# Duankaiwen/LSNet

Measured on AMD Instinct MI355X. Metric: img/s train LSNet R-50-FPN 1333x800 bs2/GPU, higher is better.
Workload: dtype f32 (fp32-equivalent: 6 bf16 MFMA terms per product on exact 3-way operand splits, fp32 accumulate); 1 GPU; LSNet R50-FPN bbox (conv_module_type=dcn), 2 img/GPU 3x800x1344 (1333x800 padded to /32), 7 gt/img, fwd+bwd+gradient arena (the reducer's buckets, no collective on one rank)+clip35+SGD; global_batch=2, parallelism=dp1, world_size=1, memory_format=channels_last, launch=eager

## Files before the change

include/lsnet_hip.h:

```cpp
#ifndef LSNET_HIP_H_
#define LSNET_HIP_H_

#include <stdint.h>

#ifdef __cplusplus
extern "C" {
#endif

typedef struct ihipStream_t *lsn_stream_t;

typedef enum {
    LSN_OK = 0,
    LSN_ERR_INVALID = -1,
    LSN_ERR_UNSUPPORTED = -2,
    LSN_ERR_RUNTIME = -3
} lsn_status;

typedef enum { LSN_NCHW = 0, LSN_NHWC = 1 } lsn_layout;

typedef struct { int64_t b, c, h, w; } lsn_strides4;

typedef struct {
    int B, C, H, W;
    int Co, Ho, Wo;
// ... 245 lines not shown

int lsn_bn_eval_act_forward(const float *x, const float *residual, float *y, const float *running_mean,
                            const float *running_var, const float *gamma, const float *beta, float eps, int relu,
                            int N, int C, lsn_stream_t stream);
int64_t lsn_bn_eval_act_workspace_bytes(int N, int C);
int lsn_bn_eval_act_backward(const float *grad_y, const float *y, const float *x, const float *running_mean,
                             const float *running_var, const float *gamma, float eps, int relu, float *grad_x,
                             float *grad_residual, float *grad_gamma, float *grad_beta, void *workspace, int N,
                             int C, int accumulate, lsn_stream_t stream);
int lsn_relu_gate(const float *grad_y, const float *y, float *grad, int64_t n, lsn_stream_t stream);
typedef struct lsn_gate_job {
    const float *grad_y, *y;
    float *grad;
    int B;
    int64_t per_image, gy_batch_stride;
} lsn_gate_job;
int lsn_relu_gate_multi(int n_jobs, const lsn_gate_job *jobs, lsn_stream_t stream);

enum {
    LSN_DBG_BLOCK_MASK = 0xffff,
    LSN_DBG_ANCHOR_ONE_WAVE = 1 << 20,
    LSN_DBG_FWD_SK_ALWAYS = 1 << 21,
    LSN_DBG_FWD_SK_NEVER = 1 << 22,
    LSN_DBG_ATOMIC_SCATTER = 1 << 23,
    LSN_DBG_WG_COMPUTED_TAPS = 1 << 24,
    LSN_DBG_WG_SCALAR_LOADS = 1 << 25,
    LSN_DBG_GENERAL_GEMMS = 1 << 28
};
int lsn_debug_phase_clocks(long long *device_buf_512, int word);

typedef struct lsn_prof_entry {
    char name[48];
    long long launches;
    double total_ms;
    double flops;
    double bytes;
} lsn_prof_entry;
int lsn_prof_enable(int on);
int lsn_prof_read(lsn_prof_entry *out, int max_entries);

typedef struct lsn_prof_launch {
    int kind, C, Co, kh, kw, stride, pad, dil, relu, xpitch, n_levels, has_residual, has_gate;
    int B[16], H[16], W[16];
    float ms;
} lsn_prof_launch;
int lsn_prof_launch_log(int on);
int lsn_prof_read_launches(lsn_prof_launch *out, int max_entries);

int lsn_scratch_stats(long long *out4);

int lsn_wgrad_defer(int max_mbytes, lsn_stream_t stream);
int lsn_wgrad_flush(lsn_stream_t stream);

int lsn_selftest_mfma(const float *A, const float *B, float *D, int M, int N, int K, int variant,
                      lsn_stream_t stream);

int lsn_image_prep_u8(const uint8_t *src, int sh, int sw, int c, int dh, int dw, int flip_h, int flip_v,
                      const float *mean, const float *inv_std, int reverse_channels, float pad_val, float *dst,
                      int out_h, int out_w, lsn_stream_t stream);

int lsn_cross_iou_bbox_forward(const float *pred, const float *target, const uint8_t *active, const float *anchor,
                               const float *bbox_gt, const float *weight, int64_t n, float alpha, float eps,
                               float *loss_rows, lsn_stream_t stream);
int lsn_cross_iou_bbox_backward(const float *pred, const float *target, const uint8_t *active, const float *anchor,
                                const float *bbox_gt, const float *weight, const float *grad_rows, int64_t n,
                                float alpha, float eps, float *grad_pred, lsn_stream_t stream);

int lsn_cross_iou_bbox_stage_forward(const float *pred_raw, const float *gt_pts, const float *anchor3, const float *bbox_gt,
                                     const float *weight, int64_t n, float base_scale, float alpha, float eps,
                                     float *loss_rows, lsn_stream_t stream);
int lsn_cross_iou_bbox_stage_backward(const float *pred_raw, const float *gt_pts, const float *anchor3, const float *bbox_gt,
                                      const float *weight, const float *grad_rows, int64_t n, float base_scale, float alpha,
                                      float eps, float *grad_raw, lsn_stream_t stream);

int lsn_cross_iou_rows_forward(int kind, const float *pred, const float *target, const uint8_t *active, const float *anchor,
                               const float *bbox_gt, const float *vs, const float *weight, int64_t n, int ncomp, int sub,
                               float alpha, float eps, float *loss_rows, lsn_stream_t stream);
int lsn_cross_iou_rows_backward(int kind, const float *pred, const float *target, const uint8_t *active, const float *anchor,
                                const float *bbox_gt, const float *vs, const float *weight, const float *grad_rows, int64_t n,
                                int ncomp, int sub, float alpha, float eps, float *grad_pred, lsn_stream_t stream);

int lsn_pool_output_size(int in, int k, int stride, int pad, int ceil_mode);
int lsn_max_pool2d_forward(const float *x, int x_pitch, float *y, int y_pitch, uint8_t *slot, int B, int H, int W, int C, int kh,
                           int kw, int stride, int pad, lsn_stream_t stream);
int lsn_max_pool2d_backward(const float *grad_y, int gy_pitch, const uint8_t *slot, float *grad_x, int gx_pitch, int B, int H, int W,
                            int C, int kh, int kw, int stride, int pad, lsn_stream_t stream);

int lsn_avg_pool2d_forward(const float *x, int x_pitch, float *y, int y_pitch, int B, int H, int W, int C, int kh, int kw, int stride,
                           int pad, int ceil_mode, int count_include_pad, lsn_stream_t stream);
int lsn_avg_pool2d_backward(const float *grad_y, int gy_pitch, float *grad_x, int gx_pitch, int B, int H, int W, int C, int kh, int kw,
                            int stride, int pad, int ceil_mode, int count_include_pad, lsn_stream_t stream);

int lsn_upsample_add_forward(const float *top, int top_pitch, const float *lat, int lat_pitch, float *out, int out_pitch, int B, int h,
                             int w, int H, int W, int C, lsn_stream_t stream);
int lsn_upsample_add_backward(const float *grad_out, int go_pitch, float *grad_top, int gt_pitch, int accumulate, int B, int h, int w,
                              int H, int W, int C, lsn_stream_t stream);

int lsn_corner_pool_forward(int mode, const float *x, int x_pitch, float *y, int y_pitch, int accumulate, int B, int H, int W, int C,
                            lsn_stream_t stream);
int lsn_corner_pool_backward(int mode, const float *x, int x_pitch, const float *grad_y, int gy_pitch, float *grad_x, int gx_pitch,
                             int accumulate, int B, int H, int W, int C, lsn_stream_t stream);

#ifdef __cplusplus
}
#endif
#endif
// ... 1 lines not shown
```

lsnet_amd/_lib.py:

```python
import ctypes
import os

_HERE = os.path.dirname(os.path.abspath(__file__))
SO_PATH = os.environ.get('LSNET_HIP_SO') or os.path.join(_HERE, 'csrc', 'liblsnet_hip.so')

c_float_p = ctypes.POINTER(ctypes.c_float)
c_i64_p = ctypes.POINTER(ctypes.c_int64)


class Strides4(ctypes.Structure):
    _fields_ = [('b', ctypes.c_int64), ('c', ctypes.c_int64), ('h', ctypes.c_int64), ('w', ctypes.c_int64)]


class DcnShape(ctypes.Structure):
    _fields_ = [('B', ctypes.c_int), ('C', ctypes.c_int), ('H', ctypes.c_int), ('W', ctypes.c_int),
                ('Co', ctypes.c_int), ('Ho', ctypes.c_int), ('Wo', ctypes.c_int),
                ('kh', ctypes.c_int), ('kw', ctypes.c_int), ('stride', ctypes.c_int), ('pad', ctypes.c_int),
                ('dil', ctypes.c_int), ('groups', ctypes.c_int), ('deformable_groups', ctypes.c_int),
                ('scale_h', ctypes.c_float), ('scale_w', ctypes.c_float), ('mask_is_logit', ctypes.c_int),
                ('workspace', ctypes.c_void_p), ('gather_workspace', ctypes.c_void_p),
                ('gather_workspace_bytes', ctypes.c_int64), ('accumulate_param_grads', ctypes.c_int),
                ('out_pitch', ctypes.c_int), ('weights_prepared', ctypes.c_int)]


# ... 28 lines not shown


class ConvLevel(ctypes.Structure):
    _fields_ = [('x', ctypes.c_void_p), ('out', ctypes.c_void_p), ('grad_out', ctypes.c_void_p),
                ('B', ctypes.c_int), ('H', ctypes.c_int), ('W', ctypes.c_int), ('residual', ctypes.c_void_p),
                ('gate', ctypes.c_void_p)]


class ConvWprep(ctypes.Structure):
    _fields_ = [('kind', ctypes.c_int), ('w', ctypes.c_void_p), ('prepared', ctypes.c_void_p), ('C', ctypes.c_int),
                ('Co', ctypes.c_int), ('kh', ctypes.c_int), ('kw', ctypes.c_int), ('stride', ctypes.c_int),
                ('pad', ctypes.c_int), ('dil', ctypes.c_int),
                ('bn_gamma', ctypes.c_void_p), ('bn_var', ctypes.c_void_p), ('bn_beta', ctypes.c_void_p),
                ('bn_mean', ctypes.c_void_p), ('shift_out', ctypes.c_void_p), ('bn_eps', ctypes.c_float)]


class GnLevel(ctypes.Structure):
    _fields_ = [('x', ctypes.c_void_p), ('y', ctypes.c_void_p), ('dy', ctypes.c_void_p), ('dx', ctypes.c_void_p),
                ('B', ctypes.c_int), ('HW', ctypes.c_int), ('y_batch_stride', ctypes.c_longlong),
                ('dy_batch_stride', ctypes.c_longlong)]


class GateJob(ctypes.Structure):
    _fields_ = [('grad_y', ctypes.c_void_p), ('y', ctypes.c_void_p), ('grad', ctypes.c_void_p), ('B', ctypes.c_int),
                ('per_image', ctypes.c_int64), ('gy_batch_stride', ctypes.c_int64)]


class ProfEntry(ctypes.Structure):
    _fields_ = [('name', ctypes.c_char * 48), ('launches', ctypes.c_longlong), ('total_ms', ctypes.c_double),
                ('flops', ctypes.c_double), ('bytes', ctypes.c_double)]


class ProfLaunch(ctypes.Structure):
    _fields_ = [(k, ctypes.c_int) for k in ('kind', 'C', 'Co', 'kh', 'kw', 'stride', 'pad', 'dil', 'relu', 'xpitch', 'n_levels',
                                            'has_residual', 'has_gate')] + \
               [('B', ctypes.c_int * 16), ('H', ctypes.c_int * 16), ('W', ctypes.c_int * 16), ('ms', ctypes.c_float)]


EXPORTS = [
    'lsn_last_error', 'lsn_version', 'lsn_dcn_forward', 'lsn_dcn_backward', 'lsn_dcn_backward_workspace_bytes', 'lsn_dcn_pitched_ok', 'lsn_dcn_prepared_ok',
    'lsn_deform_conv_forward', 'lsn_deform_conv_backward_input', 'lsn_deform_conv_backward_parameters',
    'lsn_modulated_deform_conv_forward', 'lsn_modulated_deform_conv_backward',
    'lsn_pyramid_deform_conv_forward', 'lsn_pyramid_deform_conv_backward_input',
    'lsn_pyramid_deform_conv_backward_parameters',
    'lsn_sigmoid_focal_loss_forward', 'lsn_sigmoid_focal_loss_backward', 'lsn_sigmoid_focal_loss_sum',
    'lsn_sigmoid_focal_loss_backward_weighted', 'lsn_sigmoid_focal_loss_level_sums', 'lsn_sigmoid_focal_loss_backward_levels',
    'lsn_level_sums', 'lsn_level_expand',
    'lsn_nms_workspace_bytes', 'lsn_nms', 'lsn_topk_columns', 'lsn_offset_chain_forward', 'lsn_offset_chain_backward', 'lsn_clip_sgd_workspace_bytes', 'lsn_clip_sgd_step', 'lsn_selftest_mfma', 'lsn_debug_phase_clocks',
    'lsn_prof_enable', 'lsn_prof_read', 'lsn_prof_launch_log', 'lsn_prof_read_launches', 'lsn_scratch_stats', 'lsn_wgrad_defer', 'lsn_wgrad_flush',
    'lsn_group_norm_workspace_bytes', 'lsn_group_norm_forward', 'lsn_group_norm_backward',
    'lsn_set_math_mode', 'lsn_get_math_mode', 'lsn_conv2d_forward', 'lsn_conv2d_forward_pitched', 'lsn_conv2d_backward_data',
    'lsn_conv2d_prepared_bytes', 'lsn_conv2d_prepare_weights', 'lsn_conv2d_prepare_weights_multi',
    'lsn_conv2d_prepare_weights_item',
    'lsn_conv2d_forward_prepared',
    'lsn_conv2d_backward_data_prepared',
    'lsn_conv2d_forward_multi', 'lsn_conv2d_backward_data_multi', 'lsn_conv2d_backward_weight_multi', 'lsn_conv2d_backward_weight',
    'lsn_grouped_conv2d_forward', 'lsn_grouped_conv2d_backward_data', 'lsn_grouped_conv2d_backward_weight',
    'lsn_bn_eval_act_forward', 'lsn_bn_eval_act_backward', 'lsn_bn_eval_act_workspace_bytes',
    'lsn_relu_gate', 'lsn_relu_gate_multi', 'lsn_conv2d_backward_weight_bn', 'lsn_conv2d_backward_weight_bn_jobs',
    'lsn_image_prep_u8', 'lsn_cross_iou_bbox_forward', 'lsn_cross_iou_bbox_backward',
    'lsn_cross_iou_bbox_stage_forward', 'lsn_cross_iou_bbox_stage_backward',
    'lsn_cross_iou_rows_forward', 'lsn_cross_iou_rows_backward',
    'lsn_assign_workspace_bytes', 'lsn_centroid_assign', 'lsn_centroid_assign_batch', 'lsn_atss_assign', 'lsn_atss_assign_batch',
    'lsn_dense_targets',
    'lsn_pool_output_size', 'lsn_max_pool2d_forward', 'lsn_max_pool2d_backward', 'lsn_avg_pool2d_forward', 'lsn_avg_pool2d_backward',
    'lsn_upsample_add_forward', 'lsn_upsample_add_backward', 'lsn_corner_pool_forward', 'lsn_corner_pool_backward',
]

_lib = None


def load():
    global _lib
    if _lib is not None:
        return _lib
    if not os.path.exists(SO_PATH):
        raise RuntimeError(
            f'{SO_PATH} is missing: build it with `python -c "import __graft_entry__ as g; g.build()"` '
            '(hipcc --offload-arch=gfx950). lsnet_amd has no fallback path.')
    lib = ctypes.CDLL(SO_PATH)
    lib.lsn_last_error.restype = ctypes.c_char_p
    lib.lsn_nms_workspace_bytes.restype = ctypes.c_int64
    lib.lsn_assign_workspace_bytes.restype = ctypes.c_int64
    lib.lsn_group_norm_workspace_bytes.restype = ctypes.c_int64
    lib.lsn_bn_eval_act_workspace_bytes.restype = ctypes.c_int64
    lib.lsn_dcn_backward_workspace_bytes.restype = ctypes.c_int64
    lib.lsn_clip_sgd_workspace_bytes.restype = ctypes.c_int64
    lib.lsn_conv2d_prepared_bytes.restype = ctypes.c_int64
    for name in EXPORTS:
        getattr(lib, name)
    _lib = lib
    return lib


def check(rc):
    if rc != 0:
        msg = load().lsn_last_error().decode('utf-8', 'replace')
        if rc == -2:
            raise NotImplementedError(msg)
        raise RuntimeError(msg)


PROF_FAMILIES = ('dcn_fwd', 'dcn_bwd_data', 'dcn_wgrad', 'conv_fwd', 'conv_bwd_data', 'conv_wgrad', 'norm', 'gconv')


def prof_enable(on, families=None):
    mask = 0
    if on:
        mask = 1 if families is None else sum(1 << PROF_FAMILIES.index(f) for f in families)
        if mask == 1 and families is not None:
            mask |= 1 << 31
    check(load().lsn_prof_enable(mask))


def prof_read():
    arr = (ProfEntry * 16)()
    n = load().lsn_prof_read(arr, 16)
    if n < 0:
        check(n)
    return {arr[i].name.decode(): dict(launches=int(arr[i].launches), total_ms=arr[i].total_ms,
                                       flops=arr[i].flops, bytes=arr[i].bytes) for i in range(n)}


def wgrad_defer(max_mbytes, stream=None):
    import ctypes
    import torch
    st = ctypes.c_void_p(torch.cuda.current_stream().cuda_stream if stream is None else stream)
    check(load().lsn_wgrad_defer(int(max_mbytes), st))


def wgrad_flush(stream=None):
    import ctypes
    import torch
    st = ctypes.c_void_p(torch.cuda.current_stream().cuda_stream if stream is None else stream)
    check(load().lsn_wgrad_flush(st))


def scratch_stats():
    import ctypes
    out = (ctypes.c_longlong * 4)()
    check(load().lsn_scratch_stats(out))
    return dict(mallocs=int(out[0]), held_bytes=int(out[1]), blocking_syncs=int(out[2]), pool_allocs=int(out[3]))


DBG_BLOCK_MASK = 0xffff
DBG_ANCHOR_ONE_WAVE = 1 << 20
DBG_FWD_SK_ALWAYS = 1 << 21
DBG_FWD_SK_NEVER = 1 << 22
DBG_ATOMIC_SCATTER = 1 << 23
DBG_WG_COMPUTED_TAPS = 1 << 24
DBG_WG_SCALAR_LOADS = 1 << 25
DBG_GENERAL_GEMMS = 1 << 28


def set_debug_word(word, buf=None):
    check(load().lsn_debug_phase_clocks(None if buf is None else ctypes.c_void_p(buf), ctypes.c_int(word)))


MATH_FP32, MATH_BF16X3, MATH_BF16X6, MATH_BF16 = 0, 1, 2, 3
_MODES = {'fp32': MATH_FP32, 'bf16x3': MATH_BF16X3, 'bf16x6': MATH_BF16X6, 'bf16': MATH_BF16}


def set_math_mode(mode):
    check(load().lsn_set_math_mode(_MODES[mode] if isinstance(mode, str) else mode))


def get_math_mode():
    m = load().lsn_get_math_mode()
    return {v: k for k, v in _MODES.items()}[m]


def split_math():
    return get_math_mode() != 'fp32'
```

lsnet_amd/csrc/build.py:

```python
import os
import shutil
import subprocess
import sys

HERE = os.path.dirname(os.path.abspath(__file__))
SO = os.path.join(HERE, 'liblsnet_hip.so')
SOURCES = ['dcn.hip', 'misc.hip', 'norm.hip', 'conv.hip', 'gconv.hip', 'image.hip', 'loss.hip', 'assign.hip', 'pool.hip']
HEADERS = ['common.h', 'dcn_kernels.h', 'dcn_gather_kernels.h', 'dcn_grouped_kernels.h', 'conv_kernels.h', 'conv_wgrad_kernels.h', 'dcn_mm_kernels.h', 'prof.h', 'cross_iou_row.h', 'assign_rows.h', 'pool_rows.h', os.path.join('..', '..', 'include', 'lsnet_hip.h')]
FLAGS = ['--offload-arch=gfx950', '-O3', '-std=c++17', '-fPIC', '-shared', '-ffp-contract=fast',
         '-fno-slp-vectorize', '-Wno-unused-result']


def kernel_signature():
    import hashlib
    h = hashlib.sha256()
    for f in ('common.h', 'conv_kernels.h', 'conv_wgrad_kernels.h', 'conv.hip', 'dcn_kernels.h', 'dcn_gather_kernels.h', 'dcn_mm_kernels.h', 'dcn_grouped_kernels.h', 'dcn.hip'):
        with open(os.path.join(HERE, f), 'rb') as fh:
            h.update(fh.read())
    return h.hexdigest()[:16]


def _hipcc():
    for c in (shutil.which('hipcc'), '/opt/rocm/bin/hipcc'):
        if c and os.path.exists(c):
            return c
    raise RuntimeError('hipcc not found: liblsnet_hip.so cannot be built')


OBJ_DIR = os.path.join(HERE, 'build')
UNIT_HEADERS = {
    'dcn.hip': ['common.h', 'dcn_kernels.h', 'dcn_gather_kernels.h', 'dcn_mm_kernels.h', 'dcn_grouped_kernels.h', 'conv_kernels.h', 'prof.h'],
    'conv.hip': ['common.h', 'conv_kernels.h', 'conv_wgrad_kernels.h', 'prof.h'],
    'misc.hip': ['common.h', 'prof.h'], 'norm.hip': ['common.h', 'prof.h'], 'gconv.hip': ['common.h', 'prof.h'],
    'image.hip': ['common.h'], 'loss.hip': ['common.h', 'cross_iou_row.h'], 'assign.hip': ['common.h', 'assign_rows.h'],
    'pool.hip': ['common.h', 'pool_rows.h'],
}
UNIT_FLAGS = {'assign.hip': ['-ffp-contract=off']}
API_HEADER = os.path.join('..', '..', 'include', 'lsnet_hip.h')


def _stale(target, deps):
    if not os.path.exists(target):
        return True
    t = os.path.getmtime(target)
    return any(os.path.exists(d) and os.path.getmtime(d) > t for d in deps)


def _unit_deps(src):
    return [os.path.join(HERE, f) for f in [src] + UNIT_HEADERS.get(src, HEADERS) + [API_HEADER]] + [os.path.abspath(__file__)]


def needs_build(so=None, obj_dir=None):
    so = so or SO
    obj_dir = obj_dir or OBJ_DIR
    if not os.path.exists(so):
        return True
    return any(_stale(os.path.join(obj_dir, s + '.o'), _unit_deps(s)) for s in SOURCES) or \
        _stale(so, [os.path.join(obj_dir, s + '.o') for s in SOURCES])


def build(force=False, verbose=False, defines=(), so=None):
    so = so or SO
    obj_dir = OBJ_DIR if so == SO else so + '.build'
    if not force and not needs_build(so, obj_dir):
        return so
    os.makedirs(obj_dir, exist_ok=True)
    cc = _hipcc()
    cflags = [f for f in FLAGS if f != '-shared'] + ['-D' + d for d in defines]
    jobs = []
    for s in SOURCES:
        obj = os.path.join(obj_dir, s + '.o')
        if force or _stale(obj, _unit_deps(s)):
            cmd = [cc] + cflags + UNIT_FLAGS.get(s, []) + ['-c', os.path.join(HERE, s), '-o', obj]
            if verbose:
                print(' '.join(cmd), file=sys.stderr)
            jobs.append((s, subprocess.Popen(cmd, cwd=HERE)))
    failed = [s for s, p in jobs if p.wait() != 0]
    if failed:
        raise RuntimeError('hipcc failed for ' + ', '.join(failed))
    cmd = [cc, '--offload-arch=gfx950', '-shared', '-fPIC'] + [os.path.join(obj_dir, s + '.o') for s in SOURCES] + ['-o', so]
    if verbose:
        print(' '.join(cmd), file=sys.stderr)
    subprocess.check_call(cmd, cwd=HERE)
    return so

# ... 26 lines not shown
```

lsnet_amd/csrc/conv.hip:

```cpp
#include <hip/hip_runtime.h>
#include <stdint.h>
#include <stdlib.h>
#include <string.h>

#include <vector>

#include "../../include/lsnet_hip.h"
#include "common.h"
#include "conv_kernels.h"
#include "conv_wgrad_kernels.h"
#include "prof.h"

namespace lsn {

int split_np();
static int conv_np()
{
    switch (split_np()) {
    case 0: return 6;
    case 1: return 1;
    case 3: return 3;
    case 6: return 6;
    default: return -1;
    }
}
static int conv_npl() { return split_npl(conv_np()); }

static long long g_stat[4] = {0, 0, 0, 0};
void lib_stat(int which, long long add) { g_stat[which & 3] += add; }

struct Scratch {
    hipStream_t st;
    float *p;
    size_t floats;
};
static Scratch g_scr[16];
static int g_nscr = 0;
struct RJob {
    bool fold;
    const float *part, *part_b;
    float *gw, *gb;
    size_t n;
    int nb, splits, splits_b, R, Co;
    WgFold f;
};
struct Arena {
    hipStream_t st;
    float *p;
    size_t floats, used;
    long long defer_mb;
    std::vector<RJob> *jobs;
};
static Arena g_arena[16];
static int g_narena = 0;
static Arena *arena_of(hipStream_t st, bool create)
{
    for (int i = 0; i < g_narena; ++i)
        if (g_arena[i].st == st) return &g_arena[i];
    if (!create || g_narena == 16) return nullptr;
    g_arena[g_narena] = Arena{st, nullptr, 0, 0, 0, new std::vector<RJob>()};
    return &g_arena[g_narena++];
}
// ... 170 lines not shown
            LSN_HIP(hipFuncSetAttribute(reinterpret_cast<const void *>(k), hipFuncAttributeMaxDynamicSharedMemorySize, (int)lds));
            attr_set = true;
        }
        hipLaunchKernelGGL(k, grid, dim3(256), lds, st, a);
    } else {
        auto k = conv_mm_kernel<TM, TN, WM, WN, NP, UNAL, FINE, TRANS, false>;
        static bool attr_set = false;
        if (!attr_set) {
            LSN_HIP(hipFuncSetAttribute(reinterpret_cast<const void *>(k), hipFuncAttributeMaxDynamicSharedMemorySize, (int)lds));
            attr_set = true;
        }
        hipLaunchKernelGGL(k, grid, dim3(256), lds, st, a);
    }
    if (ks > 1) {
        const int blocks = (int)((n / 4 + 255) / 256 < 1024 ? (n / 4 + 255) / 256 : 1024);
        const size_t o = (size_t)pix0 * a.Co;
        hipLaunchKernelGGL(conv_splitk_reduce_kernel, dim3(blocks > 0 ? blocks : 1), dim3(256), 0, st, a.part, a.lv[0].out + o, a.bias,
                           a.lv[0].res ? a.lv[0].res + o : nullptr, a.lv[0].gate ? a.lv[0].gate + o : nullptr, (int)n, a.Co, ks,
                           a.relu);
    }
    LSN_HIP(hipGetLastError());
    return 0;
}

template <int TM, int TN, int WM, int WN, int NP, bool UNAL, bool FINE, bool TRANS = false>
static int launch_conv_cfg(ConvArgs &a, int ks, hipStream_t st)
{
    constexpr int BM = WM * TM * 32, BN = WN * TN * 32;
    int tiles = 0;
    for (int i = 0; i < a.nlv; ++i) {
        a.lv[i].tile0 = tiles;
        tiles += (a.lv[i].P + BM - 1) / BM;
    }
    a.ntiles = tiles;
    return launch_conv_range<TM, TN, WM, WN, NP, UNAL, FINE, TRANS>(a, ks, 0, tiles, st);
}

template <int TM, int TN, int WM, int WN, bool FINE>
static int launch_conv(ConvArgs &a, int ks, hipStream_t st)
{
    if constexpr (TN == 2 && WN == 2) {
        if (a.C % 4 != 0 || a.xpitch % 4 != 0)
            return split_dispatch(conv_np(), [&](auto np) {
                return launch_conv_cfg<TM, TN, WM, WN, decltype(np)::value, true, false>(a, ks, st);
            });
    }
    if (a.C % 4 != 0 || a.xpitch % 4 != 0)
        return fail(LSN_ERR_UNSUPPORTED, "conv2d: C %% 4 != 0 needs more than 64 output channels");
    return split_dispatch(conv_np(), [&](auto np) {
        return launch_conv_cfg<TM, TN, WM, WN, decltype(np)::value, false, FINE>(a, ks, st);
    });
}

static int conv_forward(ConvArgs &a, hipStream_t st)
{
    auto blocks = [&](int bm, int bn) {
        int t = 0;
        for (int i = 0; i < a.nlv; ++i) t += (a.lv[i].P + bm - 1) / bm;
        return t * ((a.Co + bn - 1) / bn);
    };
    int cfg;
    if (a.Co <= 32) cfg = 4;
    else if (a.Co <= 64) cfg = 3;
    else cfg = 2;
    if (a.Co % 256 == 0 && a.C % 4 == 0 && a.xpitch % 4 == 0 && (a.kh * a.kw > 1 || blocks(64, 256) >= 512)) cfg = 5;
    const int nb = cfg == 2 ? blocks(64, 128) : cfg == 3 ? blocks(128, 64) : cfg == 5 ? blocks(64, 256) : blocks(128, 32);
    const int Tall = a.kh * a.kw * cv_ncc(a.C);
    int ks = 1;
    if (a.nlv == 1 && !a.ostep) ks = z_split(nb, Tall);
    switch (cfg) {
    case 2: return launch_conv<1, 2, 2, 2, true>(a, ks, st);
    case 3: return launch_conv<1, 2, 4, 1, false>(a, ks, st);
    case 5: return launch_conv<2, 2, 1, 4, true>(a, ks, st);
    default: return launch_conv<1, 1, 4, 1, false>(a, ks, st);
    }
}

int conv_mm_rows(int n, const float *const *x, float *const *out, const int *rows, int Cr, int xpitch, int N,
                 const unsigned short *wf, hipStream_t st)
{
    LSN_CHECK(n >= 1 && n <= CV_MAXLV && Cr % 4 == 0 && xpitch % 4 == 0 && xpitch >= Cr, "conv_mm_rows: bad arguments");
    ConvArgs a = {};
    a.nlv = n;
    for (int i = 0; i < n; ++i) {
        ConvLvl &L = a.lv[i];
        L.x = x[i], L.out = out[i], L.res = nullptr;
        L.B = 1, L.H = 1, L.W = rows[i], L.Ho = 1, L.Wo = rows[i], L.P = rows[i];
    }
    a.wf = wf;
    a.wf_bytes = (int)cv_wfrag_bytes(N, 1, Cr, conv_npl());
    a.C = Cr, a.Co = N, a.kh = a.kw = 1, a.stride = 1, a.pad_h = a.pad_w = 0, a.dil = 1;
    a.xpitch = xpitch;
    bool rows32 = true;
    for (int i = 0; i < n; ++i) rows32 = rows32 && (long long)rows[i] * N * 4 < (1ll << 31) - 256;
    if (N % 256 == 0 && rows32) {
        return split_dispatch(conv_np(), [&](auto np) {
            return launch_conv_cfg<2, 2, 1, 4, decltype(np)::value, false, true, true>(a, 1, st);
        });
    }
    return conv_forward(a, st);
}

struct BnFold {
    const float *gamma = nullptr, *var = nullptr, *beta = nullptr, *mean = nullptr;
    float *shift_out = nullptr;
    float eps = 0.f;
};

// ... 541 lines not shown
    const size_t bytes = jobs.size() * sizeof(WfragJob);
    const bool same = jobs.size() == g_jobs_host.size() && memcmp(jobs.data(), g_jobs_host.data(), bytes) == 0;
    if (!same) {
        if (jobs.size() > g_jobs_cap) {
            LSN_HIP(hipMalloc(reinterpret_cast<void **>(&g_jobs_dev), (jobs.size() + 64) * sizeof(WfragJob)));
            lib_stat(STAT_MALLOCS, 1), lib_stat(STAT_HELD_BYTES, (long long)((jobs.size() + 64) * sizeof(WfragJob)));
            g_jobs_cap = jobs.size() + 64;
        }
        LSN_HIP(hipStreamSynchronize(st));
        lib_stat(STAT_BLOCKING_SYNCS, 1);
        LSN_HIP(hipMemcpy(g_jobs_dev, jobs.data(), bytes, hipMemcpyHostToDevice));
        g_jobs_host = jobs;
    }
    const int blocks = (int)((total + 255) / 256 < 4096 ? (total + 255) / 256 : 4096);
    if (int rc = split_dispatch(conv_np(), [&](auto np) {
            hipLaunchKernelGGL(conv_wfrag_multi_kernel<SplitCfg<decltype(np)::value>::NPL>, dim3(blocks), dim3(256), 0, st, g_jobs_dev,
                               (int)jobs.size(), total);
            return 0;
        }))
        return rc;
    LSN_HIP(hipGetLastError());
    return 0;
}

}

extern "C" {

int lsn_wgrad_defer(int max_mbytes, lsn_stream_t stream)
{
    hipStream_t st = reinterpret_cast<hipStream_t>(stream);
    lsn::Arena *ar = lsn::arena_of(st, max_mbytes > 0);
    if (!ar) return max_mbytes > 0 ? lsn::fail(LSN_ERR_RUNTIME, "scratch: more than 16 streams use the library") : 0;
    if (max_mbytes > 0) {
        ar->jobs->clear();
        ar->used = 0;
        ar->defer_mb = max_mbytes;
        return 0;
    }
    const int rc = lsn::wgrad_flush(ar);
    ar->defer_mb = 0, ar->used = 0;
    return rc;
}

int lsn_wgrad_flush(lsn_stream_t stream)
{
    lsn::Arena *ar = lsn::arena_of(reinterpret_cast<hipStream_t>(stream), false);
    if (!ar) return 0;
    const int rc = lsn::wgrad_flush(ar);
    ar->used = 0;
    return rc;
}

int lsn_scratch_stats(long long *out4)
{
    LSN_CHECK(out4 != nullptr, "lsn_scratch_stats: NULL pointer");
    for (int i = 0; i < 4; ++i) out4[i] = lsn::g_stat[i];
    return 0;
}

int lsn_conv2d_backward_weight_bn(const float *x, const float *g, const float *w, const float *bn_gamma, const float *bn_mean,
                                  const float *bn_var, float bn_eps, float *grad_w, float *grad_gamma, float *grad_beta, int B,
                                  int H, int W, int C, int Co, int kh, int kw, int stride, int pad, int dil, int accumulate,
                                  lsn_stream_t stream)
{
    LSN_CHECK(x && g && w && bn_gamma && bn_mean && bn_var && grad_w && grad_gamma && grad_beta,
              "conv2d backward-weight (folded norm): NULL pointer");
    if (((size_t)kh * kw * C) % 4 != 0)
        return lsn::fail(LSN_ERR_UNSUPPORTED, "conv2d backward-weight (folded norm): kh * kw * C %% 4 != 0");
    lsn::WgFoldJobs f = {};
    f.f[0] = lsn::WgFold{w, bn_gamma, bn_mean, bn_var, grad_gamma, grad_beta, bn_eps};
    f.gw[0] = grad_w, f.njobs = 1;
    lsn::g_wg_fold = &f;
    const int rc = lsn_conv2d_backward_weight(x, g, grad_w, grad_beta, B, H, W, C, Co, kh, kw, stride, pad, dil, accumulate, stream);
    lsn::g_wg_fold = nullptr;
    return rc;
}

int lsn_conv2d_backward_weight_bn_jobs(int n_jobs, const lsn_wgrad_bn_job *jobs, int B, int H, int W, int C, int Co, int kh, int kw,
                                       int stride, int pad, int dil, int accumulate, lsn_stream_t stream)
{
    LSN_CHECK(n_jobs >= 1 && n_jobs <= 8 && jobs, "conv2d backward-weight jobs: 1 .. 8 jobs");
    lsn::WgFoldJobs f = {};
    lsn_conv_level lv[8] = {};
    for (int j = 0; j < n_jobs; ++j) {
        const lsn_wgrad_bn_job &q = jobs[j];
        LSN_CHECK(q.x && q.g && q.w && q.bn_gamma && q.bn_mean && q.bn_var && q.grad_w && q.grad_gamma && q.grad_beta,
                  "conv2d backward-weight jobs: NULL pointer in job %d", j);
        f.f[j] = lsn::WgFold{q.w, q.bn_gamma, q.bn_mean, q.bn_var, q.grad_gamma, q.grad_beta, q.bn_eps};
        f.gw[j] = q.grad_w;
        lv[j].x = q.x, lv[j].grad_out = q.g, lv[j].B = B, lv[j].H = H, lv[j].W = W;
    }
    f.njobs = n_jobs;
    int rc = 1;
    if (n_jobs > 1 && ((size_t)kh * kw * C) % 4 == 0) {
        lsn::g_wg_fold = &f;
        rc = lsn::conv_wgrad_mm(n_jobs, lv, jobs[0].grad_w, jobs[0].grad_beta, C, Co, kh, kw, stride, pad, dil, accumulate,
                                reinterpret_cast<hipStream_t>(stream));
        lsn::g_wg_fold = nullptr;
    }
    if (rc != 1) return rc;
    for (int j = 0; j < n_jobs; ++j) {
        const lsn_wgrad_bn_job &q = jobs[j];
        if (int r = lsn_conv2d_backward_weight_bn(q.x, q.g, q.w, q.bn_gamma, q.bn_mean, q.bn_var, q.bn_eps, q.grad_w, q.grad_gamma,
                                                  q.grad_beta, B, H, W, C, Co, kh, kw, stride, pad, dil, accumulate, stream))
            return r;
// ... 101 lines not shown
```

Baseline: 66.04 img/s.

## Add specialized narrow-channel 3x3 conv kernels with LDS halo tiling

Adds two dedicated 3x3 stride-1 convolution kernels. One handles narrow outputs (Co<=32, such as offset/cls heads), using an 8x16 spatial tile with a halo staged in LDS and double-buffered over input-channel chunks. The other handles narrow inputs (C<=32) feeding wide outputs, staging the input tile once and looping over 128-channel output groups. The conv forward dispatcher routes matching shapes to these kernels, which are meant to replace generic implicit-GEMM tiles that waste work when one channel dimension is small. This adds a lot of new hand-scheduled code with its own edge-case and out-of-bounds handling.

```diff
diff --git a/include/lsnet_hip.h b/include/lsnet_hip.h
--- a/include/lsnet_hip.h
+++ b/include/lsnet_hip.h
@@ -321,6 +321,8 @@
 int lsn_wgrad_defer(int max_mbytes, lsn_stream_t stream);
 int lsn_wgrad_flush(lsn_stream_t stream);
 
+int lsn_conv2d_narrow_route(int pass, int C, int Co, int kh, int kw, int stride, int pad, int dil);
+
 int lsn_selftest_mfma(const float *A, const float *B, float *D, int M, int N, int K, int variant,
                       lsn_stream_t stream);
 
diff --git a/lsnet_amd/_lib.py b/lsnet_amd/_lib.py
--- a/lsnet_amd/_lib.py
+++ b/lsnet_amd/_lib.py
@@ -104,7 +104,7 @@
     'lsn_set_math_mode', 'lsn_get_math_mode', 'lsn_conv2d_forward', 'lsn_conv2d_forward_pitched', 'lsn_conv2d_backward_data',
     'lsn_conv2d_prepared_bytes', 'lsn_conv2d_prepare_weights', 'lsn_conv2d_prepare_weights_multi',
     'lsn_conv2d_prepare_weights_item',
-    'lsn_conv2d_forward_prepared',
+    'lsn_conv2d_forward_prepared', 'lsn_conv2d_narrow_route',
     'lsn_conv2d_backward_data_prepared',
     'lsn_conv2d_forward_multi', 'lsn_conv2d_backward_data_multi', 'lsn_conv2d_backward_weight_multi', 'lsn_conv2d_backward_weight',
     'lsn_grouped_conv2d_forward', 'lsn_grouped_conv2d_backward_data', 'lsn_grouped_conv2d_backward_weight',
@@ -188,6 +188,10 @@
     check(load().lsn_wgrad_flush(st))
 
 
+def conv2d_narrow_route(pass_, C, Co, kh, kw, stride, pad, dil):
+    return bool(load().lsn_conv2d_narrow_route(int(pass_), int(C), int(Co), int(kh), int(kw), int(stride), int(pad), int(dil)))
+
+
 def scratch_stats():
     import ctypes
     out = (ctypes.c_longlong * 4)()
diff --git a/lsnet_amd/csrc/build.py b/lsnet_amd/csrc/build.py
--- a/lsnet_amd/csrc/build.py
+++ b/lsnet_amd/csrc/build.py
@@ -6,7 +6,7 @@
 HERE = os.path.dirname(os.path.abspath(__file__))
 SO = os.path.join(HERE, 'liblsnet_hip.so')
 SOURCES = ['dcn.hip', 'misc.hip', 'norm.hip', 'conv.hip', 'gconv.hip', 'image.hip', 'loss.hip', 'assign.hip', 'pool.hip']
-HEADERS = ['common.h', 'dcn_kernels.h', 'dcn_gather_kernels.h', 'dcn_grouped_kernels.h', 'conv_kernels.h', 'conv_wgrad_kernels.h', 'dcn_mm_kernels.h', 'prof.h', 'cross_iou_row.h', 'assign_rows.h', 'pool_rows.h', os.path.join('..', '..', 'include', 'lsnet_hip.h')]
+HEADERS = ['common.h', 'dcn_kernels.h', 'dcn_gather_kernels.h', 'dcn_grouped_kernels.h', 'conv_kernels.h', 'conv_narrow_kernels.h', 'conv_wgrad_kernels.h', 'dcn_mm_kernels.h', 'prof.h', 'cross_iou_row.h', 'assign_rows.h', 'pool_rows.h', os.path.join('..', '..', 'include', 'lsnet_hip.h')]
 FLAGS = ['--offload-arch=gfx950', '-O3', '-std=c++17', '-fPIC', '-shared', '-ffp-contract=fast',
          '-fno-slp-vectorize', '-Wno-unused-result']
 
@@ -14,7 +14,7 @@
 def kernel_signature():
     import hashlib
     h = hashlib.sha256()
-    for f in ('common.h', 'conv_kernels.h', 'conv_wgrad_kernels.h', 'conv.hip', 'dcn_kernels.h', 'dcn_gather_kernels.h', 'dcn_mm_kernels.h', 'dcn_grouped_kernels.h', 'dcn.hip'):
+    for f in ('common.h', 'conv_kernels.h', 'conv_narrow_kernels.h', 'conv_wgrad_kernels.h', 'conv.hip', 'dcn_kernels.h', 'dcn_gather_kernels.h', 'dcn_mm_kernels.h', 'dcn_grouped_kernels.h', 'dcn.hip'):
         with open(os.path.join(HERE, f), 'rb') as fh:
             h.update(fh.read())
     return h.hexdigest()[:16]
@@ -30,7 +30,7 @@
 OBJ_DIR = os.path.join(HERE, 'build')
 UNIT_HEADERS = {
     'dcn.hip': ['common.h', 'dcn_kernels.h', 'dcn_gather_kernels.h', 'dcn_mm_kernels.h', 'dcn_grouped_kernels.h', 'conv_kernels.h', 'prof.h'],
-    'conv.hip': ['common.h', 'conv_kernels.h', 'conv_wgrad_kernels.h', 'prof.h'],
+    'conv.hip': ['common.h', 'conv_kernels.h', 'conv_narrow_kernels.h', 'conv_wgrad_kernels.h', 'prof.h'],
     'misc.hip': ['common.h', 'prof.h'], 'norm.hip': ['common.h', 'prof.h'], 'gconv.hip': ['common.h', 'prof.h'],
     'image.hip': ['common.h'], 'loss.hip': ['common.h', 'cross_iou_row.h'], 'assign.hip': ['common.h', 'assign_rows.h'],
     'pool.hip': ['common.h', 'pool_rows.h'],
diff --git a/lsnet_amd/csrc/conv.hip b/lsnet_amd/csrc/conv.hip
--- a/lsnet_amd/csrc/conv.hip
+++ b/lsnet_amd/csrc/conv.hip
@@ -8,6 +8,7 @@
 #include "../../include/lsnet_hip.h"
 #include "common.h"
 #include "conv_kernels.h"
+#include "conv_narrow_kernels.h"
 #include "conv_wgrad_kernels.h"
 #include "prof.h"
 
@@ -284,8 +285,93 @@
     });
 }
 
+static bool narrow_fwd_shape_ok(int C, int Co, int kh, int kw, int stride, int pad_h, int pad_w, int dil, int np)
+{
+    return kh == 3 && kw == 3 && stride == 1 && dil == 1 && pad_h == 1 && pad_w == 1 && Co >= 1 && Co <= 32 && C >= 32 && C % 32 == 0 &&
+           C <= 4096 && (np == 1 || np == 3 || np == 6);
+}
+static bool narrow_fwd_args_ok(const ConvArgs &a)
+{
+    if (!narrow_fwd_shape_ok(a.C, a.Co, a.kh, a.kw, a.stride, a.pad_h, a.pad_w, a.dil, conv_np())) return false;
+    if (a.xpitch != a.C || a.ostep != 0) return false;
+    long long blocks = 0;
+    for (int i = 0; i < a.nlv; ++i) {
+        const ConvLvl &L = a.lv[i];
+        if (L.Ho != L.H || L.Wo != L.W) return false;
+        if ((long long)L.B * L.H * L.W * a.C * 4 >= NR_OOB || (long long)L.P * a.Co * 4 >= NR_OOB) return false;
+        blocks += nr_blocks(L.B, L.Ho, L.Wo);
+    }
+    return blocks < (1ll << 30);
+}
+
+static bool narrow_red_shape_ok(int C, int Co, int kh, int kw, int stride, int pad_h, int pad_w, int dil, int np)
+{
+    return kh == 3 && kw == 3 && stride == 1 && dil == 1 && pad_h == 1 && pad_w == 1 && C >= 1 && C <= 32 && Co >= 128 && Co % 128 == 0 &&
+           (np == 1 || np == 3 || np == 6);
+}
+static bool narrow_red_args_ok(const ConvArgs &a)
+{
+    if (!narrow_red_shape_ok(a.C, a.Co, a.kh, a.kw, a.stride, a.pad_h, a.pad_w, a.dil, conv_np())) return false;
+    if (a.xpitch < a.C || a.ostep != 0) return false;
+    long long blocks = 0;
+    for (int i = 0; i < a.nlv; ++i) {
+        const ConvLvl &L = a.lv[i];
+        if (L.Ho != L.H || L.Wo != L.W) return false;
+        if ((long long)L.B * L.H * L.W * a.xpitch * 4 >= NR_OOB || (long long)L.P * a.Co * 4 >= NR_OOB) return false;
+        blocks += nr_blocks(L.B, L.Ho, L.Wo);
+    }
+    return blocks < (1ll << 30);
+}
+
+static int launch_narrow_fwd(ConvArgs &a, hipStream_t st)
+{
+    int blocks = 0;
+    for (int i = 0; i < a.nlv; ++i) {
+        a.lv[i].tile0 = blocks;
+        blocks += nr_blocks(a.lv[i].B, a.lv[i].Ho, a.lv[i].Wo);
+    }
+    a.ntiles = blocks;
+    a.ksplit = 1;
+    return split_dispatch(conv_np(), [&](auto np) {
+        constexpr int NP = decltype(np)::value;
+        const size_t lds = nr_fwd_lds(SplitCfg<NP>::NPL);
+        auto k = conv_narrow_fwd_kernel<NP>;
+        static bool attr_set = false;
+        if (!attr_set) {
+            LSN_HIP(hipFuncSetAttribute(reinterpret_cast<const void *>(k), hipFuncAttributeMaxDynamicSharedMemorySize, (int)lds));
+            attr_set = true;
+        }
+        hipLaunchKernelGGL(k, dim3(blocks), dim3(128), lds, st, a);
+        LSN_HIP(hipGetLastError());
+        return 0;
+    });
+}
+
+static int launch_narrow_red(ConvArgs &a, hipStream_t st)
+{
+    int blocks = 0;
+    for (int i = 0; i < a.nlv; ++i) {
+        a.lv[i].tile0 = blocks;
+        blocks += nr_blocks(a.lv[i].B, a.lv[i].Ho, a.lv[i].Wo);
+    }
+    a.ntiles = blocks;
+    a.ksplit = 1;
+    return split_dispatch(conv_np(), [&](auto np) {
+        constexpr int NP = decltype(np)::value;
+        const size_t lds = nr_red_lds(SplitCfg<NP>::NPL);
+        bool epi = false;
+        for (int i = 0; i < a.nlv; ++i) epi = epi || a.lv[i].res || a.lv[i].gate;
+        if (epi) hipLaunchKernelGGL((conv_narrow_red_kernel<NP, true>), dim3(blocks), dim3(256), lds, st, a);
+        else hipLaunchKernelGGL((conv_narrow_red_kernel<NP, false>), dim3(blocks), dim3(256), lds, st, a);
+        LSN_HIP(hipGetLastError());
+        return 0;
+    });
+}
+
 static int conv_forward(ConvArgs &a, hipStream_t st)
 {
+    if (narrow_fwd_args_ok(a)) return launch_narrow_fwd(a, st);
+    if (narrow_red_args_ok(a)) return launch_narrow_red(a, st);
     auto blocks = [&](int bm, int bn) {
         int t = 0;
         for (int i = 0; i < a.nlv; ++i) t += (a.lv[i].P + bm - 1) / bm;
@@ -933,6 +1019,13 @@
     return rc;
 }
 
+int lsn_conv2d_narrow_route(int pass, int C, int Co, int kh, int kw, int stride, int pad, int dil)
+{
+    if (pass == 0) return lsn::narrow_fwd_shape_ok(C, Co, kh, kw, stride, pad, pad, dil, lsn::conv_np()) ? 1 : 0;
+    if (pass == 1) return lsn::narrow_red_shape_ok(Co, C, kh, kw, stride, pad, pad, dil, lsn::conv_np()) ? 1 : 0;
+    return 0;
+}
+
 int lsn_scratch_stats(long long *out4)
 {
     LSN_CHECK(out4 != nullptr, "lsn_scratch_stats: NULL pointer");
diff --git a/lsnet_amd/csrc/conv_narrow_kernels.h b/lsnet_amd/csrc/conv_narrow_kernels.h
--- /dev/null
+++ b/lsnet_amd/csrc/conv_narrow_kernels.h
@@ -0,0 +1,338 @@
+#pragma once
+#include <hip/hip_runtime.h>
+#include <stdint.h>
+
+#include "common.h"
+#include "conv_kernels.h"
+
+namespace lsn {
+
+constexpr int NR_BH = 8, NR_BW = 16;
+constexpr int NR_PH = NR_BH + 2, NR_PW = NR_BW + 2;
+constexpr int NR_PITCH = 20;
+constexpr int NR_PLANE = NR_PH * NR_PITCH * 64;
+constexpr int NR_OOB = 0x7fff0000;
+
+__host__ __device__ inline int nr_blocks(int B, int Ho, int Wo) { return B * ((Ho + NR_BH - 1) / NR_BH) * ((Wo + NR_BW - 1) / NR_BW); }
+inline size_t nr_fwd_lds(int npl) { return (size_t)2 * npl * NR_PLANE; }
+
+template <int NP>
+__global__ __launch_bounds__(128) void conv_narrow_fwd_kernel(const ConvArgs a)
+{
+    using SC = SplitCfg<NP>;
+    constexpr int NPL = SC::NPL;
+    constexpr int BUF = NPL * NR_PLANE;
+    constexpr int NITEM = NR_PH * NR_PW * 8;
+    constexpr int NLD = (NITEM + 127) / 128;
+    constexpr int FRAG = 2 * NPL * 1024;
+    extern __shared__ __align__(16) unsigned char smem[];
+
+    const int tid = threadIdx.x, lane = tid & 63, wave = tid >> 6;
+    const int blk = xcd_remap((int)blockIdx.x, a.ntiles);
+    int li = 0;
+    while (li + 1 < a.nlv && blk >= a.lv[li + 1].tile0) ++li;
+    const ConvLvl &L = a.lv[li];
+    const int nbx = (L.Wo + NR_BW - 1) / NR_BW, nby = (L.Ho + NR_BH - 1) / NR_BH;
+    int rem = blk - L.tile0;
+    const int b = rem / (nby * nbx);
+    rem -= b * nby * nbx;
+    const int by = rem / nbx, bx = rem - by * nbx;
+    const int oy0 = by * NR_BH, ox0 = bx * NR_BW;
+    const int ncc = a.C >> 5;
+
+    const __amdgpu_buffer_rsrc_t xrs =
+        __builtin_amdgcn_make_buffer_rsrc(const_cast<float *>(L.x), 0, L.B * L.H * L.W * a.C * 4, 0x00020000);
+    const __amdgpu_buffer_rsrc_t wrs =
+        __builtin_amdgcn_make_buffer_rsrc(const_cast<unsigned short *>(a.wf), 0, a.wf_bytes, 0x00020000);
+
+    int goff[NLD], woff[NLD];
+#pragma unroll
+    for (int ps = 0; ps < NLD; ++ps) {
+        const int item = ps * 128 + tid;
+        const int pp = item >> 3, c4 = item & 7;
+        const int prow = pp / NR_PW, pcol = pp - prow * NR_PW;
+        const int y = oy0 - 1 + prow, x = ox0 - 1 + pcol;
+        const bool ok = item < NITEM && (unsigned)y < (unsigned)L.H && (unsigned)x < (unsigned)L.W;
+        goff[ps] = ok ? (((b * L.H + y) * L.W + x) * a.C + 4 * c4) * 4 : NR_OOB;
+        woff[ps] = (prow * NR_PITCH + pcol) * 64 + ((((c4 >> 1) ^ ((pcol >> 2) & 3)) << 4) | ((c4 & 1) << 3));
+    }
+    float4 xv[NLD];
+    auto issue_x = [&](int cc, bool live) {
+#pragma unroll
+        for (int ps = 0; ps < NLD; ++ps) xv[ps] = cv_load4(xrs, live ? goff[ps] + cc * 128 : NR_OOB, 0);
+    };
+    auto commit_slice = [&](int ps, unsigned char *buf) {
+        unsigned p0[NPL], p1[NPL];
+        split_planes<NPL>(xv[ps].x, xv[ps].y, p0);
+        split_planes<NPL>(xv[ps].z, xv[ps].w, p1);
+        if (NLD * 128 == NITEM || ps + 1 < NLD || tid < NITEM - (NLD - 1) * 128) {
+#pragma unroll
+            for (int q = 0; q < NPL; ++q) *reinterpret_cast<uint2 *>(buf + q * NR_PLANE + woff[ps]) = make_uint2(p0[q], p1[q]);
+        }
+    };
+
+    const int prow0 = wave * 4 + ((lane >> 4) & 1), pcol0 = lane & 15;
+    int xoff[3][2];
+#pragma unroll
+    for (int j = 0; j < 3; ++j)
+#pragma unroll
+        for (int ks = 0; ks < 2; ++ks)
+            xoff[j][ks] = (prow0 * NR_PITCH + pcol0 + j) * 64 + (((ks * 2 + (lane >> 5)) ^ (((pcol0 + j) >> 2) & 3)) << 4);
+
+    bf16x8 Xf[2][2][NPL];
+    bf16x8 Wf[3][NPL];
+    auto read_x = [&](const unsigned char *buf, int s) {
+        const int tap = s >> 1, ks = s & 1, i = tap / 3, j = tap - i * 3;
+#pragma unroll
+        for (int t = 0; t < 2; ++t)
+#pragma unroll
+            for (int q = 0; q < NPL; ++q)
+                Xf[s & 1][t][q] =
+                    *reinterpret_cast<const bf16x8 *>(buf + q * NR_PLANE + (i + 2 * t) * (NR_PITCH * 64) + xoff[j][ks]);
+    };
+    auto issue_w = [&](int cc, int s) {
+        const int tap = s >> 1, ks = s & 1;
+        const int soff = (tap * ncc + cc) * FRAG;
+#pragma unroll
+        for (int q = 0; q < NPL; ++q) Wf[s % 3][q] = cv_load_frag(wrs, lane * 16 + (ks * NPL + q) * 1024, soff);
+    };
+
+    f32x16 acc[2];
+#pragma unroll
+    for (int t = 0; t < 2; ++t)
+#pragma unroll
+        for (int r = 0; r < 16; ++r) acc[t][r] = 0.f;
+
+    issue_x(0, true);
+    issue_w(0, 0);
+    issue_w(0, 1);
+#pragma unroll
+    for (int ps = 0; ps < NLD; ++ps) commit_slice(ps, smem);
+    __syncthreads();
+
+    for (int cc = 0; cc < ncc; ++cc) {
+        const unsigned char *bc = smem + (cc & 1) * BUF;
+        unsigned char *bn = smem + ((cc & 1) ^ 1) * BUF;
+        const bool more = cc + 1 < ncc;
+        issue_x(cc + 1, more);
+        read_x(bc, 0);
+        __builtin_amdgcn_sched_barrier(0);
+#pragma unroll
+        for (int s = 0; s < 18; ++s) {
+            if (s + 2 < 18) issue_w(cc, s + 2);
+            else issue_w(more ? cc + 1 : cc, s + 2 - 18);
+            if (s + 1 < 18) read_x(bc, s + 1);
+#pragma unroll
+            for (int prod = 0; prod < NP; ++prod)
+#pragma unroll
+                for (int t = 0; t < 2; ++t)
+                    acc[t] = mfma_bf16(Xf[s & 1][t][SC::pa(prod)], Wf[s % 3][SC::pb(prod)], acc[t]);
+            constexpr int S0 = 18 - NLD;
+            if (s >= S0 && s - S0 < NLD) commit_slice(s - S0, bn);
+            __builtin_amdgcn_sched_barrier(0);
+        }
+        __syncthreads();
+    }
+
+    const int co = lane & 31;
+    const int out_bytes = L.P * a.Co * 4;
+    const bool cok = co < a.Co;
+    float bias = 0.f;
+    if (a.bias != nullptr && cok) bias = a.bias[co];
+    const __amdgpu_buffer_rsrc_t ors = __builtin_amdgcn_make_buffer_rsrc(L.out, 0, out_bytes, 0x00020000);
+    const __amdgpu_buffer_rsrc_t rrs =
+        __builtin_amdgcn_make_buffer_rsrc(const_cast<float *>(L.res ? L.res : L.out), 0, out_bytes, 0x00020000);
+    const __amdgpu_buffer_rsrc_t grs =
+        __builtin_amdgcn_make_buffer_rsrc(const_cast<float *>(L.gate ? L.gate : L.out), 0, out_bytes, 0x00020000);
+    const bool has_res = L.res != nullptr, has_gate = L.gate != nullptr;
+#pragma unroll
+    for (int t = 0; t < 2; ++t) {
+        int off[16];
+        float rv[16], gv[16];
+#pragma unroll
+        for (int r = 0; r < 16; ++r) {
+            const int m = mfma32_row(r, lane);
+            const int oy = oy0 + wave * 4 + 2 * t + (m >> 4), ox = ox0 + (m & 15);
+            off[r] = cok && oy < L.Ho && ox < L.Wo ? (((b * L.Ho + oy) * L.Wo + ox) * a.Co + co) * 4 : NR_OOB;
+            rv[r] = 0.f, gv[r] = 1.f;
+        }
+        if (has_res)
+#pragma unroll
+            for (int r = 0; r < 16; ++r) rv[r] = __builtin_bit_cast(float, __builtin_amdgcn_raw_buffer_load_b32(rrs, off[r], 0, 0));
+        if (has_gate)
+#pragma unroll
+            for (int r = 0; r < 16; ++r) gv[r] = __builtin_bit_cast(float, __builtin_amdgcn_raw_buffer_load_b32(grs, off[r], 0, 0));
+#pragma unroll
+        for (int r = 0; r < 16; ++r) {
+            float v = acc[t][r] + bias;
+            if (has_res) v += rv[r];
+            if (a.relu) v = fmaxf(v, 0.f);
+            if (has_gate) v = gv[r] > 0.f ? v : 0.f;
+            __builtin_amdgcn_raw_buffer_store_b32(__float_as_uint(v), ors, off[r], 0, 0);
+        }
+    }
+}
+
+
+inline size_t nr_red_lds(int npl) { return (size_t)npl * NR_PLANE; }
+
+template <int NP, bool EPI>
+__global__ __launch_bounds__(256, 2) void conv_narrow_red_kernel(const ConvArgs a)
+{
+    using SC = SplitCfg<NP>;
+    constexpr int NPL = SC::NPL;
+    constexpr int NITEM = NR_PH * NR_PW * 16;
+    constexpr int NLD = (NITEM + 255) / 256;
+    constexpr int FRAG = 2 * NPL * 1024;
+    extern __shared__ __align__(16) unsigned char smem[];
+
+    const int tid = threadIdx.x, lane = tid & 63, wave = tid >> 6;
+    const int wp = wave & 1, wc = wave >> 1;
+    const int blk = xcd_remap((int)blockIdx.x, a.ntiles);
+    int li = 0;
+    while (li + 1 < a.nlv && blk >= a.lv[li + 1].tile0) ++li;
+    const ConvLvl &L = a.lv[li];
+    const int nbx = (L.Wo + NR_BW - 1) / NR_BW, nby = (L.Ho + NR_BH - 1) / NR_BH;
+    int rem = blk - L.tile0;
+    const int b = rem / (nby * nbx);
+    rem -= b * nby * nbx;
+    const int by = rem / nbx, bx = rem - by * nbx;
+    const int oy0 = by * NR_BH, ox0 = bx * NR_BW;
+    const int NT = cv_nt(a.Co);
+
+    const __amdgpu_buffer_rsrc_t xrs =
+        __builtin_amdgcn_make_buffer_rsrc(const_cast<float *>(L.x), 0, L.B * L.H * L.W * a.xpitch * 4, 0x00020000);
+    const __amdgpu_buffer_rsrc_t wrs =
+        __builtin_amdgcn_make_buffer_rsrc(const_cast<unsigned short *>(a.wf), 0, a.wf_bytes, 0x00020000);
+
+    bf16x8 Wf[2][2][NPL];
+    const int wvoff = lane * 16 + wc * 2 * FRAG;
+    auto issue_w = [&](int h, int s) {
+        const int tap = s >> 1, ks = s & 1;
+        const int soff = (tap * NT + h * 4) * FRAG;
+#pragma unroll
+        for (int j = 0; j < 2; ++j)
+#pragma unroll
+            for (int q = 0; q < NPL; ++q) Wf[s & 1][j][q] = cv_load_frag(wrs, wvoff + j * FRAG + (ks * NPL + q) * 1024, soff);
+    };
+
+    {
+        float v0[NLD], v1[NLD];
+        int woff[NLD];
+#pragma unroll
+        for (int ps = 0; ps < NLD; ++ps) {
+            const int item = ps * 256 + tid;
+            const int pp = item >> 4, cp = item & 15;
+            const int prow = pp / NR_PW, pcol = pp - prow * NR_PW;
+            const int y = oy0 - 1 + prow, x = ox0 - 1 + pcol;
+            const bool ok = item < NITEM && (unsigned)y < (unsigned)L.H && (unsigned)x < (unsigned)L.W;
+            const int g = (((b * L.H + y) * L.W + x) * a.xpitch + 2 * cp) * 4;
+            v0[ps] = __builtin_bit_cast(float, __builtin_amdgcn_raw_buffer_load_b32(xrs, ok && 2 * cp < a.C ? g : NR_OOB, 0, 0));
+            v1[ps] = __builtin_bit_cast(float, __builtin_amdgcn_raw_buffer_load_b32(xrs, ok && 2 * cp + 1 < a.C ? g + 4 : NR_OOB, 0, 0));
+            woff[ps] = (prow * NR_PITCH + pcol) * 64 + ((((cp >> 2) ^ ((pcol >> 2) & 3)) << 4) | ((cp & 3) << 2));
+        }
+        issue_w(0, 0);
+#pragma unroll
+        for (int ps = 0; ps < NLD; ++ps) {
+            unsigned p[NPL];
+            split_planes<NPL>(v0[ps], v1[ps], p);
+            if (NLD * 256 == NITEM || ps + 1 < NLD || tid < NITEM - (NLD - 1) * 256) {
+#pragma unroll
+                for (int q = 0; q < NPL; ++q) *reinterpret_cast<unsigned *>(smem + q * NR_PLANE + woff[ps]) = p[q];
+            }
+        }
+    }
+    __syncthreads();
+
+    const int prow0 = wp * 4 + ((lane >> 4) & 1), pcol0 = lane & 15;
+    int xoff[3][2];
+#pragma unroll
+    for (int j = 0; j < 3; ++j)
+#pragma unroll
+        for (int ks = 0; ks < 2; ++ks)
+            xoff[j][ks] = (prow0 * NR_PITCH + pcol0 + j) * 64 + (((ks * 2 + (lane >> 5)) ^ (((pcol0 + j) >> 2) & 3)) << 4);
+    bf16x8 Xf[2][2][NPL];
+    auto read_x = [&](int s) {
+        const int tap = s >> 1, ks = s & 1, i = tap / 3, j = tap - i * 3;
+#pragma unroll
+        for (int t = 0; t < 2; ++t)
+#pragma unroll
+            for (int q = 0; q < NPL; ++q)
+                Xf[s & 1][t][q] =
+                    *reinterpret_cast<const bf16x8 *>(smem + q * NR_PLANE + (i + 2 * t) * (NR_PITCH * 64) + xoff[j][ks]);
+    };
+
+    const int out_bytes = L.P * a.Co * 4;
+    const __amdgpu_buffer_rsrc_t ors = __builtin_amdgcn_make_buffer_rsrc(L.out, 0, out_bytes, 0x00020000);
+    const bool has_gate = EPI && L.gate != nullptr;
+    const int nh = a.Co >> 7;
+    read_x(0);
+    for (int h = 0; h < nh; ++h) {
+        f32x16 acc[2][2];
+#pragma unroll
+        for (int t = 0; t < 2; ++t)
+#pragma unroll
+            for (int j = 0; j < 2; ++j)
+#pragma unroll
+                for (int r = 0; r < 16; ++r) acc[t][j][r] = 0.f;
+        __builtin_amdgcn_sched_barrier(0);
+#pragma unroll
+        for (int s = 0; s < 18; ++s) {
+            if (s + 1 < 18) issue_w(h, s + 1);
+            else issue_w(h + 1 < nh ? h + 1 : h, 0);
+            read_x(s + 1 < 18 ? s + 1 : 0);
+#pragma unroll
+            for (int prod = 0; prod < NP; ++prod)
+#pragma unroll
+                for (int t = 0; t < 2; ++t)
+#pragma unroll
+                    for (int j = 0; j < 2; ++j)
+                        acc[t][j] = mfma_bf16(Xf[s & 1][t][SC::pa(prod)], Wf[s & 1][j][SC::pb(prod)], acc[t][j]);
+            __builtin_amdgcn_sched_barrier(0);
+        }
+        const int eHo = L.Ho, eWo = L.Wo, eCo = a.Co;
+        const int xl = eWo - ox0 - 4 * (lane >> 5);
+        int colbad[8];
+#pragma unroll
+        for (int k = 0; k < 8; ++k) colbad[k] = ((xl - 1 - ((k & 3) + 8 * (k >> 2))) >> 31) & NR_OOB;
+#pragma unroll
+        for (int j = 0; j < 2; ++j) {
+            const int c = h * 128 + wc * 64 + j * 32 + (lane & 31);
+            const float bias = a.bias != nullptr ? a.bias[c] : 0.f;
+#pragma unroll
+            for (int t = 0; t < 2; ++t) {
+                const int oyt = oy0 + wp * 4 + 2 * t;
+                const int pb = (((b * eHo + oyt) * eWo + ox0 + 4 * (lane >> 5)) * eCo + c) * 4;
+                int voff[16], soff[16];
+                float rv[16], gv[16];
+#pragma unroll
+                for (int r = 0; r < 16; ++r) {
+                    const int cr = (r & 3) + 8 * ((r >> 2) & 1), row = r >> 3;
+                    voff[r] = pb | colbad[(r & 3) + 4 * ((r >> 2) & 1)] | (oyt + row < eHo ? 0 : NR_OOB);
+                    soff[r] = (row * eWo + cr) * eCo * 4;
+                    rv[r] = 0.f, gv[r] = 1.f;
+                }
+                if constexpr (EPI) {
+                    const __amdgpu_buffer_rsrc_t rrs = __builtin_amdgcn_make_buffer_rsrc(
+                        const_cast<float *>(L.res ? L.res : L.out), 0, L.res ? out_bytes : 0, 0x00020000);
+#pragma unroll
+                    for (int r = 0; r < 16; ++r) rv[r] = __builtin_bit_cast(float, __builtin_amdgcn_raw_buffer_load_b32(rrs, voff[r], soff[r], 0));
+                    const __amdgpu_buffer_rsrc_t grs = __builtin_amdgcn_make_buffer_rsrc(
+                        const_cast<float *>(L.gate ? L.gate : L.out), 0, L.gate ? out_bytes : 0, 0x00020000);
+#pragma unroll
+                    for (int r = 0; r < 16; ++r) gv[r] = __builtin_bit_cast(float, __builtin_amdgcn_raw_buffer_load_b32(grs, voff[r], soff[r], 0));
+                }
+#pragma unroll
+                for (int r = 0; r < 16; ++r) {
+                    float v = acc[t][j][r] + bias;
+                    if constexpr (EPI) v += rv[r];
+                    if (a.relu) v = fmaxf(v, 0.f);
+                    if constexpr (EPI) v = (gv[r] > 0.f || !has_gate) ? v : 0.f;
+                    __builtin_amdgcn_raw_buffer_store_b32(__float_as_uint(v), ors, voff[r], soff[r], 0);
+                }
+            }
+        }
+    }
+}
+
+}
```

Result: no change. 66.39 img/s, median of 6 (+0.5%).
